# eritpchy/video-subtitle-extractor

Measured on AMD Instinct MI355X. Metric: OCR frames/sec (det+rec) @1080p, higher is better.
Workload: dtype f16

## Files before the change

### __graft_entry__.py

```python
import os
import subprocess
import sys

ROOT = os.path.dirname(os.path.abspath(__file__))
PKG = os.path.join(ROOT, "video-subtitle-extractor_amd")
CSRC = os.path.join(PKG, "csrc")
LIB = os.path.join(PKG, "libvse_hip.so")
HIP_SOURCES = ["vse_runtime.hip", "conv_select.hip", "conv_mfma.hip", "conv_gemm.hip", "conv_patch.hip", "conv_col.hip", "conv_c3.hip", "conv_pw.hip", "conv_dwpw.hip", "conv_smallm.hip", "conv_head.hip", "conv_stem.hip", "simple_ops.hip", "lstm.hip", "prepost.hip", "chain.hip", "frame_change.hip", "audio_match.hip"]


def _newer(target, deps):
    if not os.path.exists(target):
        return True
    t = os.path.getmtime(target)
    return any(os.path.getmtime(d) > t for d in deps)


def build(force=False):
    hipcc = os.environ.get("HIPCC", "/opt/rocm/bin/hipcc")
    srcs = [os.path.join(CSRC, s) for s in HIP_SOURCES]
    deps = srcs + [os.path.join(CSRC, "common.h"), os.path.join(CSRC, "conv_common.h"), os.path.join(CSRC, "db_geometry.h"),
                   os.path.join(ROOT, "include", "vse_hip.h")]
    if force or _newer(LIB, deps):
        objs = []
        os.makedirs(os.path.join(CSRC, "build"), exist_ok=True)
        procs = []
        for s in srcs:
            o = os.path.join(CSRC, "build", os.path.basename(s) + ".o")
            objs.append(o)
            if force or _newer(o, [s] + deps[len(srcs):]):
                cmd = [hipcc, "--offload-arch=gfx950", "-O3", "-std=c++17", "-fPIC", "-ffp-contract=off", "-c", s, "-o", o]
                procs.append((cmd, subprocess.Popen(cmd)))
        for cmd, p in procs:
            if p.wait() != 0:
                raise RuntimeError("hipcc failed: " + " ".join(cmd))
        cmd = [hipcc, "--offload-arch=gfx950", "-shared", "-fPIC", "-o", LIB] + objs
        subprocess.check_call(cmd)
    sys.path.insert(0, ROOT)
    import vse_amd
    from vse_amd import engine
    engine.load_library()
# ... 53 lines not shown
```

### video-subtitle-extractor_amd/csrc/conv_common.h

```cpp
#pragma once
#include "common.h"

#define PTW 32
#define CTW 32
#define CPW 48
#define C3BN 64
#define PW_MAXN 256
#define PW_MAXN_HILO 128
#define DWPW_ROWS_MAX_KS 3
#define DWPW_ROWS_MAX_KS_S1 3

struct ConvParams {
    const half_t* in;
    const half_t* w;
    const float* bias;
    const half_t* res;
    const half_t* zero;
    void* out;
    int H, W, Hs, Ws, in_ld, cinp, inshift;
    int OH, OW;
    long M;
    int kh, kw, sh, sw, ph, pw;
    int Np, nk;
    int nkh;
    int out_ld, out_f32;
    int res_ld, resshift, res_hs, res_ws;
    int act, act2;
    float act_a, act_b, post_a, post_b;
    int flags, coutp;
    unsigned ntn;
    unsigned ntiles;
    int tiles_h, tiles_w;
    const float* dotw;
    float dotb;
    int dotact, dot_f32, dot_ld;
    void* dot_out;
    const half_t* in2;
    int in2_ld, in2_shift, in2_hs, in2_ws, nv0;
    unsigned long long* trace;
    int vec16;
    long wimg_stride;
    int hw_img, tiles_img;
    const int* wl_out;
    int in_lo_off;
    int res_lo_off;
    int lo_off;
    const half_t* ogate;
    int ogate_ld;
    int wnp;
    const uint8_t* u8src;
    int u8_h, u8_w;
    long u8_pitch, u8_fstride;
    int pack_g, nimg;
    unsigned pack_mag_ow, pack_mag_d;
};

typedef const __attribute__((address_space(1))) void* gptr_t;
typedef __attribute__((address_space(3))) void* lptr_t;

__device__ __forceinline__ void glds16(const void* g, half_t* l) {
    __builtin_amdgcn_global_load_lds((gptr_t)g, (lptr_t)l, 16, 0, 0);
}

__device__ __forceinline__ void glds16_asm(const void* g, half_t* l) {
    unsigned keep;
    const unsigned dst = __builtin_amdgcn_readfirstlane((unsigned)(size_t)(lptr_t)l);
    asm volatile("s_mov_b32 %0, m0\n\ts_mov_b32 m0, %2\n\ts_nop 0\n\tglobal_load_lds_dwordx4 %1, off\n\ts_mov_b32 m0, %0"
                 : "=&s"(keep) : "v"(g), "s"(dst) : "memory");
}

#define OOB 0x80000000u
typedef __attribute__((address_space(3))) void* ldsv_t;

template <int N> __device__ __forceinline__ void wait_vm() {
    static_assert(N >= 0 && N <= 16, "vmcnt literal");
    if constexpr (N == 0) asm volatile("s_waitcnt vmcnt(0)" ::: "memory");
    else if constexpr (N == 1) asm volatile("s_waitcnt vmcnt(1)" ::: "memory");
    else if constexpr (N == 2) asm volatile("s_waitcnt vmcnt(2)" ::: "memory");
    else if constexpr (N == 3) asm volatile("s_waitcnt vmcnt(3)" ::: "memory");
    else if constexpr (N == 4) asm volatile("s_waitcnt vmcnt(4)" ::: "memory");
    else if constexpr (N == 5) asm volatile("s_waitcnt vmcnt(5)" ::: "memory");
    else if constexpr (N == 6) asm volatile("s_waitcnt vmcnt(6)" ::: "memory");
    else if constexpr (N == 7) asm volatile("s_waitcnt vmcnt(7)" ::: "memory");
    else if constexpr (N == 8) asm volatile("s_waitcnt vmcnt(8)" ::: "memory");
    else if constexpr (N == 9) asm volatile("s_waitcnt vmcnt(9)" ::: "memory");
    else if constexpr (N == 10) asm volatile("s_waitcnt vmcnt(10)" ::: "memory");
    else if constexpr (N == 11) asm volatile("s_waitcnt vmcnt(11)" ::: "memory");
// ... 167 lines not shown
    t.vlast = min(ox0 + TW, t.vw) - 1;
    t.g0 = (int)__umulhi((unsigned)ox0, p.pack_mag_ow);
    t.n0 = ox0 + p.pw * t.g0;
    t.used = TW + KW - 1 + p.pw * ((int)__umulhi((unsigned)max(t.vlast, 0), p.pack_mag_ow) - t.g0);
    return t;
}
__device__ __forceinline__ bool conv_pack_src(const ConvParams& p, const ConvPackTile& t, int px, int& g, int& ix) {
    const unsigned n = (unsigned)(t.n0 + px);
    g = (int)__umulhi(n, p.pack_mag_d);
    ix = (int)n - g * (p.W + p.pw) - p.pw;
    return px < t.used && ix >= 0 && ix < p.W && (long)g * p.OW < t.vw;
}
__device__ __forceinline__ int conv_pack_fragcol(const ConvParams& p, const ConvPackTile& t, int ox0, int v) {
    return v - ox0 + p.pw * ((int)__umulhi((unsigned)max(min(v, t.vlast), 0), p.pack_mag_ow) - t.g0);
}

__device__ __forceinline__ float conv_epilogue_dot(const ConvParams& p, const float16v& acc, const float (&bias)[16],
                                                   const float (&dotw)[16]) {
    float v[16];
#pragma unroll
    for (int e = 0; e < 16; ++e) v[e] = acc[e] + bias[e];
    vse_act_n(v, p.act, p.act_a, p.act_b);
    if (p.post_a != 1.f || p.post_b != 0.f) {
#pragma unroll
        for (int e = 0; e < 16; ++e) v[e] = v[e] * p.post_a + p.post_b;
    }
    vse_act_n(v, p.act2, 0.f, 0.f);
    float part = 0.f;
#pragma unroll
    for (int e = 0; e < 16; ++e) part += v[e] * dotw[e];
    return part;
}

enum { CK_NONE = 0, CK_GEMM, CK_SMALLM, CK_MFMA, CK_PATCH, CK_COL, CK_C3, CK_PW, CK_DWPW, CK_HEAD, CK_STEM };
struct ConvKernel {
    int family;
    int rc;
    int arg[3];
};

struct GemmCfg { int bm, bn, wm, wn, bk, st; };
constexpr GemmCfg kCfg[] = {{128, 128, 2, 2, 32, 3}, {256, 64, 4, 1, 32, 3}, {256, 32, 4, 1, 32, 3}, {256, 128, 4, 2, 32, 3},
                            {256, 256, 4, 4, 32, 3}, {256, 192, 8, 2, 32, 3}, {256, 256, 4, 4, 64, 2}, {256, 192, 8, 2, 64, 2}};

struct SrcGeom { int h, w; long pitch, fstride; };
ConvParams conv_params(const vse_op& o, const TView& in, const TView& res, const TView& in2, const TView& out, const TView& dot_out,
                       const char* wts, const half_t* zero, const int* wl_out, const uint8_t* u8src, const SrcGeom& src);
ConvKernel conv_select(const ConvParams& p, int Kp);
int conv_kernel_name(const ConvKernel& k, char* buf, size_t n);
int launch_conv(const vse_op& o, const TView& in, const TView& res, const TView& in2, const TView& out, const TView& dot_out,
                const char* wts, const half_t* zero, const int* wl_out, const uint8_t* u8src, const SrcGeom& src, hipStream_t st);
static inline long conv_images(const ConvParams& p) { return p.OH && p.OW ? p.M / ((long)p.OH * p.OW) : 0; }
int conv_pack_group(long images, int OW, int TW, int spare, int gap);
void conv_pack_plan(ConvParams& p, int TW, int spare);

int launch_conv_gemm(const ConvParams& p, const ConvKernel& k, hipStream_t st);
int launch_conv_smallm(const ConvParams& p, const ConvKernel& k, hipStream_t st);
int launch_conv_mfma(const ConvParams& p, const ConvKernel& k, hipStream_t st);
int launch_conv_patch(const ConvParams& p, const ConvKernel& k, hipStream_t st);
int launch_conv_col(const ConvParams& p, const ConvKernel& k, hipStream_t st);
int launch_conv_c3(const ConvParams& p, const ConvKernel& k, hipStream_t st);
int launch_conv_pw(const ConvParams& p, const ConvKernel& k, hipStream_t st);
int launch_conv_dwpw(const ConvParams& p, const ConvKernel& k, hipStream_t st);
int launch_conv_head(const ConvParams& p, const ConvKernel& k, hipStream_t st);
int launch_conv_stem(const ConvParams& p, const ConvKernel& k, hipStream_t st);
```

### video-subtitle-extractor_amd/csrc/conv_select.hip

```cpp
#include <stdlib.h>
#include <cstdio>
#include "conv_common.h"


static int conv_gemm_mode(int kh, int kw, int sh, int sw, int ph, int pw, int cinp, int Kp, int inshift, int flags) {
    (void)sh; (void)sw;
    if (inshift || (flags & (F_PATCH | F_DOT1 | F_SRC2))) return 0;
    if (cinp % 32) return 0;
    if (kh * kw > 31) return 0;
    if (kh < 2 * ph + 1 || kw < 2 * pw) return 0;
    if (kh == 1 && kw == 1 && ph == 0 && pw == 0 && Kp == cinp) return 2;
    return 1;
}
static bool conv_gemm_span_ok(const ConvParams& p, int Kp) {
    const double span = ((double)512 * p.sw + (512.0 / p.OW + 3) * p.sh * p.Ws + (double)p.kh * p.Ws + p.kw) * p.in_ld * 2;
    return !(span > 1.9e9 || (double)Kp * p.Np * 2 > 1.9e9);
}

static int conv_gemm_config(int Np, int cinp, long M) {
    auto ntn = [&](int bn) { return (long)((Np + bn - 1) / bn); };
    auto deep = [&](int c) { return cinp % 64 == 0 ? c + 2 : c; };
    if (Np <= 32) return 2;
    if (Np <= 64) return 1;
    const long mt = (M + 255) / 256;
// ... 225 lines not shown
    const int kt = (f & F_WK32) ? 32 : 64;
    const bool same_hw = p.H == p.OH && p.W == p.OW && p.Hs == p.H && p.Ws == p.W;
    if (conv_smallk_ok(p, same_hw)) return pick(CK_SMALLM, kt, hilo);
    const int mode = conv_gemm_mode(p.kh, p.kw, p.sh, p.sw, p.ph, p.pw, p.cinp, Kp, p.inshift, f);
    if (mode && conv_smallm_ok(p, mode, same_hw)) return pick(CK_SMALLM, kt, hilo);
    if (mode && conv_gemm_span_ok(p, Kp)) return pick(CK_GEMM, conv_gemm_config(p.Np, p.cinp, p.M), mode == 1);
    if (f & F_WK32) return refuse(VSE_E_UNSUPPORTED);
    return pick(CK_MFMA, conv_tile_bn(p.Np), p.inshift != 0);
}

int conv_kernel_name(const ConvKernel& k, char* buf, size_t n) {
    const int* a = k.arg;
    const char* tf[2] = {"false", "true"};
    if (k.rc != VSE_OK) return snprintf(buf, n, "(refused: %d)", k.rc);
    switch (k.family) {
        case CK_GEMM: {
            const GemmCfg& g = kCfg[a[0]];
            return snprintf(buf, n, "conv_gemm_kernel<%d, %d, %d, %d, %d, %d, %d>", g.bm, g.bn, g.wm, g.wn, g.bk, g.st, a[1]);
        }
        case CK_SMALLM: return snprintf(buf, n, "conv_smallm%s_kernel<%d>", a[1] ? "_hl" : "", a[0]);
        case CK_MFMA:
            return snprintf(buf, n, "conv_mfma_kernel<%d, %d, %d, %d, %s>", a[0] == 128 ? 128 : 256, a[0], a[0] == 128 ? 2 : 4, a[0] == 128 ? 2 : 1,
                            tf[a[1]]);
        case CK_PATCH: return snprintf(buf, n, "conv_patch_kernel<%d, %d, %d>", a[0], a[1], a[2]);
        case CK_COL: return snprintf(buf, n, "conv_col_kernel<%d, %d>", a[0], a[1]);
        case CK_C3: return snprintf(buf, n, "conv_c3%s_kernel<%d, %d>", a[1] ? "n32" : "", a[0], 8 / a[0]);
        case CK_PW:
            return a[2] ? snprintf(buf, n, "conv_pw_tail_kernel<%d>", a[0]) : snprintf(buf, n, "conv_pw_kernel<%d, %s>", a[0], tf[a[1]]);
        case CK_DWPW:
            return a[2] ? snprintf(buf, n, "conv_dwpw_rows_kernel<%d, %s, %d>", a[0], tf[a[1]], a[2])
                        : snprintf(buf, n, "conv_dwpw_kernel<%d, 3, %s>", a[0], tf[a[1]]);
        case CK_HEAD: return snprintf(buf, n, a[0] ? "conv_head_up2r_kernel" : "conv_head_up2_kernel");
        case CK_STEM: return snprintf(buf, n, "conv_stem_kernel<%d, %d, %s, %s>", a[0], a[0], tf[a[1]], tf[a[2]]);
        default: return snprintf(buf, n, "?");
    }
}


int launch_conv(const vse_op& o, const TView& in, const TView& res, const TView& in2, const TView& out, const TView& dot_out,
                const char* wts, const half_t* zero, const int* wl_out, const uint8_t* u8src, const SrcGeom& src, hipStream_t st) {
    const ConvParams p = conv_params(o, in, res, in2, out, dot_out, wts, zero, wl_out, u8src, src);
    const int f = p.flags, Np = p.Np, cinp = p.cinp;
    if (f & F_SRC2) {
        if (!in2.ptr || in2.esize != 2 || (in2.ld & 7) || in.c + in2.c != cinp) return VSE_E_INVAL;
        if ((in2.h << p.in2_shift) != p.H || (in2.w << p.in2_shift) != p.W) return VSE_E_INVAL;
    } else if (in.c != cinp) {
        return VSE_E_INVAL;
    }
    if (in.esize != 2 || ((in.ld & 7) && !((f & F_UP2HEAD) && in.ld == 1)) || (cinp & 7)) return VSE_E_INVAL;
    if ((f & F_RES) && (res.esize != 2 || (res.ld & 3))) return VSE_E_INVAL;
    if ((!(f & (F_DOT1 | F_ONECH)) && (out.ld & 3)) || (Np & 7)) return VSE_E_INVAL;
    if ((f & F_ONECH) && (!(f & F_PIXSHUF) || !(f & F_OUT_F32) || Np != 32 || out.ld != 1 || out.esize != 4 || (f & F_RES)))
        return VSE_E_INVAL;
    const int mul = (f & F_PIXSHUF) ? 2 : 1;
    if (out.h != p.OH * mul || out.w != p.OW * mul || out.n != in.n) return VSE_E_INVAL;
    if (p.res_lo_off && (!p.vec16 || p.resshift || (p.res_lo_off & 7))) return VSE_E_INVAL;
    if (p.lo_off && (!p.vec16 || (f & (F_OUT_F32 | F_ONECH | F_DOT1 | F_UP2HEAD)) || (p.lo_off & 7) || out.ld < p.lo_off + Np / ((f & F_PIXSHUF) ? 4 : 1)))
        return VSE_E_INVAL;
    if ((f & F_OGATE) && ((f & (F_SRC2 | F_IMGW | F_PIXSHUF | F_DOT1 | F_UP2HEAD)) || !in2.ptr || in2.esize != 2 || in2.n != in.n || in2.h != 1
                          || in2.w != 1 || in2.c < Np || (in2.ld & 7) || (reinterpret_cast<uintptr_t>(in2.ptr) & 15)))
        return VSE_E_INVAL;
    if ((f & F_U8SRC) && (!(f & F_STEM) || !p.u8src || p.u8_h <= 0 || p.u8_w <= 0)) return VSE_E_INVAL;
    if (p.wl_out && (f & (F_DOT1 | F_SRC2 | F_UP2HEAD | F_PIXSHUF))) return VSE_E_UNSUPPORTED;
    const ConvKernel k = conv_select(p, o.p[P_KTOT]);
    if (k.family == CK_NONE) return k.rc;
    if (!p.zero && !(f & (F_IMGW | F_DWPRE))) return VSE_E_INVAL;
    switch (k.family) {
        case CK_GEMM: return launch_conv_gemm(p, k, st);
// ... 12 lines not shown
```

### video-subtitle-extractor_amd/csrc/vse_runtime.hip

```cpp
#include <stdlib.h>
#include <cstdarg>
#include <cstdio>
#include <cstring>
#include <string>
#include <vector>

#include "conv_common.h"

static thread_local std::string g_err;
static void set_err(const char* fmt, ...) {
    char buf[512];
    va_list ap;
    va_start(ap, fmt);
    vsnprintf(buf, sizeof buf, fmt, ap);
    va_end(ap);
    g_err = buf;
}
void vse_set_error(const char* msg) { g_err = msg ? msg : ""; }
#define HIP_TRY(expr)                                                                  \
    do {                                                                               \
        hipError_t e_ = (expr);                                                        \
        if (e_ != hipSuccess) {                                                        \
            set_err("%s failed: %s (%s:%d)", #expr, hipGetErrorString(e_), __FILE__, __LINE__); \
            return VSE_E_HIP;                                                          \
        }                                                                              \
    } while (0)

struct vse_ctx {
    int device;
    std::vector<void*> weights;
    std::vector<size_t> weight_bytes;
    void* zero_page;
};

struct vse_plan {
    vse_ctx* ctx;
    int weights_id;
    std::vector<vse_op> ops;
    size_t ws_bytes;
    int max_ext;
    int n_levels;
    int batch;
    bool u8_source;
    int src_h, src_w;
    long src_pitch, src_fstride;
};

int vse_frame_change_launch(const void* d_bgr, int n, int64_t pitch, int64_t frame_stride, int y0, int y1, int x0, int x1, int edge_thresh,
                            void* d_state, int reset, int32_t* d_counts, void* stream);
size_t vse_audio_match_ws(const long* m, const long* n, int nq);
int vse_audio_match_launch(const uint8_t* const* pat, const uint8_t* const* win, const long* m, const long* n, int nq, void* d_ws,
                           unsigned long long* d_out, void* stream);

extern "C" {

const char* vse_last_error(void) { return g_err.c_str(); }
size_t vse_sizeof_op(void) { return sizeof(vse_op); }
size_t vse_sizeof_view(void) { return sizeof(vse_view); }
int vse_abi_version(void) { return 4; }

int vse_init(int device_id, vse_ctx** out) {
    if (!out) return VSE_E_INVAL;
    int count = 0;
    HIP_TRY(hipGetDeviceCount(&count));
    if (device_id < 0 || device_id >= count) {
        set_err("device %d not present (%d visible)", device_id, count);
        return VSE_E_INVAL;
    }
    HIP_TRY(hipSetDevice(device_id));
    hipDeviceProp_t prop;
    HIP_TRY(hipGetDeviceProperties(&prop, device_id));
// ... 85 lines not shown
            if (v->arena >= 2) p->max_ext = std::max(p->max_ext, v->arena - 2);
            if (v->arena == 0) {
                const size_t end = (size_t)v->off + ((size_t)v->n * v->h * v->w - 1) * v->ld * v->esize + (size_t)v->c * v->esize;
                if (end > ws_bytes) {
                    set_err("op %d: view exceeds workspace (%zu > %zu)", i, end, ws_bytes);
                    delete p;
                    return VSE_E_INVAL;
                }
            }
        }
        if ((size_t)o.w_off > wbytes || (size_t)o.b_off > wbytes) {
            set_err("op %d: weight offset out of range", i);
            delete p;
            return VSE_E_INVAL;
        }
        if (o.kind == OP_CHAIN) {
            int hdr[16];
            const size_t words = 16 + (size_t)std::max(o.p[4], 0) * 16 + (size_t)std::max(o.p[3], 0) * 28;
            if ((size_t)o.w_off + words * 4 > wbytes || (o.w_off & 3) ||
                hipMemcpy(hdr, reinterpret_cast<const char*>(c->weights[weights_id]) + o.w_off, sizeof hdr, hipMemcpyDeviceToHost) != hipSuccess) {
                set_err("op %d: chain descriptor out of the weight blob", i);
                delete p;
                return VSE_E_INVAL;
            }
            if (hdr[0] != 0x43484e31 || hdr[1] != o.p[3] || hdr[2] != o.p[4] || hdr[5] != o.p[2] || hdr[3] < 0 || hdr[4] < 0 ||
                (size_t)o.w_off + (size_t)hdr[4] + (size_t)hdr[3] > wbytes) {
                set_err("op %d: chain descriptor does not match its record (magic %#x, stages %d / %d, buffers %d / %d, LDS %d / %d)", i, hdr[0],
                        hdr[1], o.p[3], hdr[2], o.p[4], hdr[5], o.p[2]);
                delete p;
                return VSE_E_INVAL;
            }
        }
    }
    *out = p;
    return VSE_OK;
}

void vse_plan_destroy(vse_plan* p) { delete p; }

static inline TView resolve(const vse_view& v, char* ws, char* wts, void* const* ext) {
    TView t;
    t.ptr = nullptr;
    t.n = v.n; t.h = v.h; t.w = v.w; t.c = v.c; t.ld = v.ld; t.esize = v.esize;
    if (v.n == 0) return t;
    char* base = v.arena == 0 ? ws : (v.arena == 1 ? wts : reinterpret_cast<char*>(ext[v.arena - 2]));
    t.ptr = base + v.off;
    return t;
}

static int run_op(vse_plan* p, int i, char* ws, void* const* ext, const int32_t* wtab, hipStream_t st, const SrcGeom& src) {
    const vse_op& o = p->ops[i];
    const int* wl_in = (wtab && o.p[P_WLIN]) ? wtab + (size_t)(o.p[P_WLIN] - 1) * p->batch : nullptr;
    const int* wl_out = (wtab && o.p[P_WLOUT]) ? wtab + (size_t)(o.p[P_WLOUT] - 1) * p->batch : nullptr;
    char* wts = reinterpret_cast<char*>(p->ctx->weights[p->weights_id]);
    const TView in0 = resolve(o.in0, ws, wts, ext), in1 = resolve(o.in1, ws, wts, ext),
                in2 = resolve(o.in2, ws, wts, ext), out = resolve(o.out, ws, wts, ext),
                out2 = resolve(o.out2, ws, wts, ext);
    int rc;
    if (o.kind == OP_CONV) {
        const uint8_t* u8src = (o.flags & F_U8SRC) ? reinterpret_cast<const uint8_t*>(ext[0]) : nullptr;
        rc = launch_conv(o, in0, in1, in2, out, out2, wts, reinterpret_cast<const half_t*>(p->ctx->zero_page), wl_out, u8src, src, st);
    } else if (o.kind == OP_CHAIN) {
        rc = launch_chain(o, in0, out, out2, in2, wts, st);
    } else {
        rc = launch_simple_op(o, in0, in1, in2, out, out2, wts, wl_in, wl_out, st);
    }
    if (rc != VSE_OK) set_err("op %d (kind %d) failed to launch: rc=%d (%s)", i, o.kind, rc, hipGetErrorString(hipGetLastError()));
    return rc;
}

static int check_run(vse_plan* p, void* ws, void* const* ext, int n_ext, const int32_t* d_widths, const char* who) {
    if (!p || !ext || n_ext <= p->max_ext) {
        set_err("%s: need %d external pointers", who, p ? p->max_ext + 1 : 0);
        return VSE_E_INVAL;
    }
    if (!ws && p->ws_bytes) return VSE_E_INVAL;
    if (p->n_levels && !d_widths) {
        set_err("%s: the plan was compiled for ragged batches (%d width levels): run it with a width table", who, p->n_levels);
        return VSE_E_INVAL;
    }
    if (!p->n_levels && d_widths) {
        set_err("%s: width table given to a plan that was not compiled for ragged batches", who);
        return VSE_E_INVAL;
    }
    if (p->u8_source && (p->src_h <= 0 || p->src_w <= 0)) {
        set_err("%s: the plan pre-processes the uint8 frames in its stem: call vse_plan_set_source (or vse_det_forward) first", who);
        return VSE_E_INVAL;
    }
    return VSE_OK;
}

int vse_plan_set_source(vse_plan* p, int src_h, int src_w, int64_t pitch, int64_t frame_stride) {
// ... 199 lines not shown
    static thread_local char buf[96];
    buf[0] = 0;
    if (!op) return buf;
    const vse_op& o = *op;
    static const char* simple[] = {"", "", "dwconv_kernel", "pool_kernel", "gap_kernel", "scale_kernel", "binary_kernel", "resize_kernel",
                                   "unary_kernel", "layernorm_kernel", "attn_kernel", "softmax_kernel", "lstm_kernel", "wscale_kernel", "chain_kernel"};
    if (o.kind != OP_CONV) {
        snprintf(buf, sizeof buf, "%s", (o.kind >= 2 && o.kind <= OP_CHAIN) ? simple[o.kind] : "?");
        return buf;
    }
    auto shape = [](const vse_view& v) { return TView{nullptr, v.n, v.h, v.w, v.c, v.ld, v.esize}; };
    const ConvParams p = conv_params(o, shape(o.in0), shape(o.in1), shape(o.in2), shape(o.out), shape(o.out2), nullptr, nullptr, nullptr, nullptr,
                                     SrcGeom{0, 0, 0, 0});
    conv_kernel_name(conv_select(p, o.p[P_KTOT]), buf, sizeof buf);
    return buf;
}

int vse_plan_profile(vse_plan* p, void* ws, void* const* ext, int n_ext, const int32_t* d_widths, void* stream, float* ms) {
    if (!ms) return VSE_E_INVAL;
    int rc0 = check_run(p, ws, ext, n_ext, d_widths, "vse_plan_profile");
    if (rc0 != VSE_OK) return rc0;
    hipStream_t st = reinterpret_cast<hipStream_t>(stream);
    const int n = (int)p->ops.size();
    std::vector<hipEvent_t> ev(n + 1);
    for (auto& e : ev) HIP_TRY(hipEventCreate(&e));
    HIP_TRY(hipEventRecord(ev[0], st));
    for (int i = 0; i < n; ++i) {
        int rc = run_op(p, i, reinterpret_cast<char*>(ws), ext, d_widths, st, SrcGeom{p->src_h, p->src_w, p->src_pitch, p->src_fstride});
        if (rc != VSE_OK) return rc;
        HIP_TRY(hipEventRecord(ev[i + 1], st));
    }
    HIP_TRY(hipStreamSynchronize(st));
    for (int i = 0; i < n; ++i) HIP_TRY(hipEventElapsedTime(&ms[i], ev[i], ev[i + 1]));
    for (auto& e : ev) (void)hipEventDestroy(e);
    return VSE_OK;
}

}
```

### video-subtitle-extractor_amd/engine.py

```python
import ctypes as C
import os

import numpy as np

from . import compiler, ir

_HERE = os.path.dirname(os.path.abspath(__file__))
LIB_PATH = os.environ.get("VSE_LIB_PATH") or os.path.join(_HERE, "libvse_hip.so")

EXPORTS = [
    "vse_init", "vse_destroy", "vse_last_error", "vse_sizeof_op", "vse_sizeof_view", "vse_abi_version",
    "vse_weights_upload", "vse_weights_free", "vse_plan_create", "vse_plan_destroy", "vse_plan_run", "vse_plan_run_ragged",
    "vse_plan_width_levels", "vse_plan_profile", "vse_op_kernel_name", "vse_det_preprocess", "vse_db_workspace_bytes",
    "vse_db_postprocess", "vse_rec_preprocess", "vse_rec_preprocess_scratch_bytes", "vse_ctc_collapse", "vse_ctc_collapse_ragged",
    "vse_det_forward", "vse_rec_forward", "vse_plan_set_source", "vse_plan_takes_frames",
    "vse_rec_graph_create", "vse_graph_launch", "vse_graph_destroy", "vse_frame_change_state_bytes", "vse_frame_change",
    "vse_audio_match_workspace_bytes", "vse_audio_match",
]


class VseError(RuntimeError):
    pass


# ... 70 lines not shown
                                       C.c_void_p]
    lib.vse_db_postprocess.argtypes = [C.c_void_p, C.c_void_p, C.c_int, C.c_int, C.c_int, C.c_int, C.c_int,
                                       C.POINTER(DbParams), C.c_void_p, C.c_size_t, C.POINTER(Box), C.c_int,
                                       C.POINTER(C.c_int), C.c_void_p]
    lib.vse_rec_preprocess.argtypes = [C.c_void_p, C.c_void_p, C.c_int, C.c_int, C.c_int, C.c_int64, C.c_int64,
                                       C.POINTER(Crop), C.c_int, C.c_void_p, C.c_int, C.c_int, C.c_void_p,
                                       C.c_size_t, C.c_void_p]
    lib.vse_ctc_collapse.argtypes = [C.c_void_p, C.c_void_p, C.c_int, C.c_int, C.c_void_p, C.c_void_p, C.c_void_p,
                                     C.c_void_p]
    lib.vse_ctc_collapse_ragged.argtypes = [C.c_void_p, C.c_void_p, C.c_int, C.c_int, C.c_void_p, C.c_void_p, C.c_void_p,
                                            C.c_void_p, C.c_void_p]
    lib.vse_frame_change_state_bytes.restype = C.c_size_t
    lib.vse_frame_change_state_bytes.argtypes = [C.c_int, C.c_int]
    lib.vse_frame_change.argtypes = [C.c_void_p, C.c_void_p, C.c_int, C.c_int, C.c_int, C.c_int64, C.c_int64, C.c_int, C.c_int,
                                     C.c_int, C.c_int, C.c_int, C.c_void_p, C.c_int, C.c_void_p, C.c_void_p]
    lib.vse_audio_match_workspace_bytes.restype = C.c_size_t
    lib.vse_audio_match_workspace_bytes.argtypes = [C.c_void_p, C.c_int]
    lib.vse_audio_match.argtypes = [C.c_void_p, C.c_void_p, C.c_int64, C.c_void_p, C.c_int64, C.c_void_p, C.c_int, C.c_void_p,
                                    C.c_size_t, C.c_void_p, C.c_void_p]
    if lib.vse_sizeof_op() != ir.OP_DT.itemsize or lib.vse_sizeof_view() != ir.VIEW_DT.itemsize:
        raise VseError(f"ABI mismatch: vse_op {lib.vse_sizeof_op()} vs {ir.OP_DT.itemsize}, "
                       f"vse_view {lib.vse_sizeof_view()} vs {ir.VIEW_DT.itemsize}")
    _lib = lib
    return lib


def op_kernel_names(ops):
    lib = load_library()
    ops = np.ascontiguousarray(ops)
    base = ops.ctypes.data
    return [lib.vse_op_kernel_name(C.c_void_p(base + i * ops.itemsize)).decode() for i in range(len(ops))]


def _check(rc, what):
    if rc < 0:
        raise VseError(f"{what} failed (rc={rc}): {load_library().vse_last_error().decode(errors='replace')}")
    return rc


def _torch():
    import torch
    if not torch.cuda.is_available():
        raise VseError("no HIP device visible: the OCR hot path runs only on MI355X (gfx950); no CPU fallback")
    return torch


class Context:

    def __init__(self, device=0):
        self.lib = load_library()
        self.torch = _torch()
        self.device = device
        self.handle = C.c_void_p()
        _check(self.lib.vse_init(device, C.byref(self.handle)), "vse_init")
        self.tdev = self.torch.device("cuda", device)

    def stream(self):
        return C.c_void_p(self.torch.cuda.current_stream(self.tdev).cuda_stream)

    def streams_concurrent(self, a, b, spin_cycles=1_500_000):
        t = self.torch
        x = self.__dict__.setdefault("_probe_buf", t.zeros(64, device=self.tdev))
        for s in (a, b):
            with t.cuda.stream(s):
                x.add_(1)
        t.cuda.synchronize(self.tdev)
# ... 328 lines not shown

    def det_forward(self, frames_u8, dst_h, dst_w, slot=0):
        t = self.ctx.torch
        assert frames_u8.dtype == t.uint8 and frames_u8.dim() == 4 and frames_u8.shape[3] == 3
        assert frames_u8.stride(3) == 1 and frames_u8.stride(2) == 3
        n, h, w, _ = frames_u8.shape
        self.program(n, dst_h, dst_w)
        prog, handle = self._ensure((n, dst_h, dst_w))
        assert len(prog.outputs) == 1 and prog.outputs[0]["kind"] == "map" and prog.outputs[0]["ld"] == 1, "not a one-map detector plan"
        x = None if self.fuse_preprocess else t.empty((n, dst_h, dst_w, 8), dtype=t.float16, device=self.ctx.tdev)
        prob = t.empty((n, dst_h, dst_w), dtype=t.float32, device=self.ctx.tdev)
        ws = self._workspace((n, dst_h, dst_w), prog, slot)
        _check(self.ctx.lib.vse_det_forward(self.ctx.handle, handle, C.c_void_p(ws.data_ptr()), C.c_void_p(frames_u8.data_ptr()), n, h, w,
                                            frames_u8.stride(1), frames_u8.stride(0), dst_h, dst_w, 1 if self.input_norm is not None else 0,
                                            C.c_void_p(x.data_ptr()) if x is not None else None, C.c_void_p(prob.data_ptr()),
                                            self.ctx.stream()), "vse_det_forward")
        return prob

    def profile_frames(self, frames_u8, dst_h, dst_w, slot=0):
        if not self.fuse_preprocess:
            return self.profile(self.ctx.det_preprocess(frames_u8, dst_h, dst_w, raw=self.input_norm is not None), slot)
        t = self.ctx.torch
        n, h, w, _ = frames_u8.shape
        self.program(n, dst_h, dst_w)
        prog, handle = self._ensure((n, dst_h, dst_w))
        _check(self.ctx.lib.vse_plan_set_source(handle, h, w, frames_u8.stride(1), frames_u8.stride(0)), "vse_plan_set_source")
        outs = [t.empty((o["n"], o["h"], o["w"], o["ld"]), dtype=t.float32, device=self.ctx.tdev) for o in prog.outputs]
        ptrs = (C.c_void_p * (1 + len(outs)))(frames_u8.data_ptr(), *[o.data_ptr() for o in outs])
        ms = (C.c_float * len(prog.ops))()
        ws = self._workspace((n, dst_h, dst_w), prog, slot)
        self.last_outs = outs
        _check(self.ctx.lib.vse_plan_profile(handle, C.c_void_p(ws.data_ptr()), ptrs, len(ptrs), None, self.ctx.stream(), ms),
               "vse_plan_profile")
        names = op_kernel_names(prog.ops)
        return np.array(ms[:], dtype=np.float32), prog, names

    def rec_forward(self, x, widths=None, slot=0):
        t = self.ctx.torch
        assert x.dtype == t.float16 and x.is_contiguous() and x.shape[3] == 8
        n, h, w, _ = x.shape
        self.program(n, h, w)
        prog, handle = self._ensure((n, h, w))
        assert len(prog.outputs) == 1 and prog.outputs[0]["kind"] == "idx_maxp"
        tt = prog.outputs[0]["w"]
        wt = self._width_table(prog, widths, n, w)
        idx_maxp = t.empty((n, 1, tt, 2), dtype=t.float32, device=self.ctx.tdev)
        oi = t.zeros((n, tt), dtype=t.int32, device=self.ctx.tdev)
        ol = t.empty((n,), dtype=t.int32, device=self.ctx.tdev)
        oc = t.empty((n,), dtype=t.float32, device=self.ctx.tdev)
        ws = self._workspace((n, h, w), prog, slot)
        _check(self.ctx.lib.vse_rec_forward(self.ctx.handle, handle, C.c_void_p(ws.data_ptr()), C.c_void_p(x.data_ptr()),
                                            C.c_void_p(wt.data_ptr()) if wt is not None else None, prog.out_level,
                                            C.c_void_p(idx_maxp.data_ptr()), n, tt, C.c_void_p(oi.data_ptr()), C.c_void_p(ol.data_ptr()),
                                            C.c_void_p(oc.data_ptr()), self.ctx.stream()), "vse_rec_forward")
        return oi, ol, oc

    def rec_graph_buffers(self, n, h, w, slot=0):
        t = self.ctx.torch
        key = (n, h, w, slot)
        if not hasattr(self, "_graphs"):
            self._graphs = {}
        if key in self._graphs:
            self._graphs[key] = self._graphs.pop(key)
        else:
            self._drop_graphs(keep=self.GRAPH_CACHE_MAX - 1)
            self.program(n, h, w)
            prog, handle = self._ensure((n, h, w))
# ... 5 lines not shown
                ol=t.zeros((n,), dtype=t.int32, device=dev), oc=t.zeros((n,), dtype=t.float32, device=dev), graph=None, tt=tt,
                wsbuf=t.zeros(max(prog.ws_bytes, 256), dtype=t.uint8, device=dev), prog=prog, handle=handle)
        return self._graphs[key]

    def rec_forward_graph(self, bufs, widths):
        t = self.ctx.torch
        prog = bufs["prog"]
        self._upload_i32(prog.width_table(widths), out=bufs["wt"])
        if bufs["graph"] is None:
            g = C.c_void_p()
            n = bufs["x"].shape[0]
            _check(self.ctx.lib.vse_rec_graph_create(self.ctx.handle, bufs["handle"], C.c_void_p(bufs["wsbuf"].data_ptr()),
                                                     C.c_void_p(bufs["x"].data_ptr()), C.c_void_p(bufs["wt"].data_ptr()), prog.out_level,
                                                     C.c_void_p(bufs["idx_maxp"].data_ptr()), n, bufs["tt"], C.c_void_p(bufs["oi"].data_ptr()),
                                                     C.c_void_p(bufs["ol"].data_ptr()), C.c_void_p(bufs["oc"].data_ptr()), self.ctx.stream(),
                                                     C.byref(g)), "vse_rec_graph_create")
            bufs["graph"] = g
        _check(self.ctx.lib.vse_graph_launch(bufs["graph"], self.ctx.stream()), "vse_graph_launch")
        return bufs["oi"].clone(), bufs["ol"].clone(), bufs["oc"].clone()

    def profile(self, x, slot=0, widths=None):
        n, h, w, _ = x.shape
        self.program(n, h, w)
        prog, handle = self._ensure((n, h, w))
        outs, ptrs = self._ext(prog, x)
        ms = (C.c_float * len(prog.ops))()
        ws = self._workspace((n, h, w), prog, slot)
        wt = self._width_table(prog, widths, n, w)
        self.last_tlen = wt[prog.out_level] if wt is not None else None
        self.last_outs = outs
        _check(self.ctx.lib.vse_plan_profile(handle, C.c_void_p(ws.data_ptr()), ptrs, len(ptrs),
                                             C.c_void_p(wt.data_ptr()) if wt is not None else None, self.ctx.stream(), ms),
               "vse_plan_profile")
        variants = op_kernel_names(prog.ops)
        return np.array(ms[:], dtype=np.float32), prog, variants
```

Baseline: 2058.

## Fuse 3x3 conv with following 3x3 stride-2 max pool into one kernel

New measurement: 2088, median of 6. +1.5%, better.

```diff
diff --git a/__graft_entry__.py b/__graft_entry__.py
--- a/__graft_entry__.py
+++ b/__graft_entry__.py
@@ -6,7 +6,7 @@
 PKG = os.path.join(ROOT, "video-subtitle-extractor_amd")
 CSRC = os.path.join(PKG, "csrc")
 LIB = os.path.join(PKG, "libvse_hip.so")
-HIP_SOURCES = ["vse_runtime.hip", "conv_select.hip", "conv_mfma.hip", "conv_gemm.hip", "conv_patch.hip", "conv_col.hip", "conv_c3.hip", "conv_pw.hip", "conv_dwpw.hip", "conv_smallm.hip", "conv_head.hip", "conv_stem.hip", "simple_ops.hip", "lstm.hip", "prepost.hip", "chain.hip", "frame_change.hip", "audio_match.hip"]
+HIP_SOURCES = ["vse_runtime.hip", "conv_select.hip", "conv_mfma.hip", "conv_gemm.hip", "conv_patch.hip", "conv_col.hip", "conv_c3.hip", "conv_c3pool.hip", "conv_pw.hip", "conv_dwpw.hip", "conv_smallm.hip", "conv_head.hip", "conv_stem.hip", "simple_ops.hip", "lstm.hip", "prepost.hip", "chain.hip", "frame_change.hip", "audio_match.hip"]
 
 
 def _newer(target, deps):
diff --git a/video-subtitle-extractor_amd/csrc/conv_c3pool.hip b/video-subtitle-extractor_amd/csrc/conv_c3pool.hip
--- /dev/null
+++ b/video-subtitle-extractor_amd/csrc/conv_c3pool.hip
@@ -0,0 +1,244 @@
+#include "conv_common.h"
+
+template <int BN>
+__global__ __launch_bounds__(512, 4) void conv_c3pool_kernel(const ConvParams p) {
+    constexpr int PTH = 8, WCO = 2;
+    constexpr int TN = BN / (32 * WCO);
+    constexpr int PPIX = 352, PNPL = 3, TPS = 2, RING = 2;
+    constexpr int PW = PTW + 2, P = PW * (PTH + 2);
+    constexpr int PATCH_HALFS = PPIX * 32, WSTAGE_HALFS = TPS * BN * 32, DUMMY_HALFS = 2 * 512;
+    constexpr int NCG = BN / 8;
+    static_assert(BN == 64 || BN == 128, "cout tile");
+    static_assert(PTH * PTW * BN <= 2 * PATCH_HALFS + RING * WSTAGE_HALFS + DUMMY_HALFS, "the fp16 conv tile must fit the patch + ring");
+    __shared__ __attribute__((aligned(16))) half_t lds[2 * PATCH_HALFS + RING * WSTAGE_HALFS + DUMMY_HALFS + 2 * BN];
+    float* const sbias = reinterpret_cast<float*>(lds + 2 * PATCH_HALFS + RING * WSTAGE_HALFS + DUMMY_HALFS);
+    half_t* const patch0 = lds;
+    half_t* const ring0 = lds + 2 * PATCH_HALFS;
+    half_t* const dummy0 = ring0 + RING * WSTAGE_HALFS;
+
+    const int tid = threadIdx.x;
+    const int lane = tid & 63;
+    const int wave = __builtin_amdgcn_readfirstlane(tid >> 6);
+    const int wpx = wave / WCO, wco = wave % WCO;
+
+    const unsigned nblk = gridDim.x, bid = blockIdx.x;
+    const unsigned q8 = nblk >> 3, r8 = nblk & 7, xcd = bid & 7, slot = bid >> 3;
+    unsigned t = (xcd < r8 ? xcd * (q8 + 1) : r8 * (q8 + 1) + (xcd - r8) * q8) + slot;
+    const int nt = t % p.ntn;  t /= p.ntn;
+    const int tx = t % p.tiles_w;  t /= p.tiles_w;
+    const int seg = t % p.pool_nseg;
+    const long img = t / p.pool_nseg;
+    const int ox0 = tx * (PTW - 2) - 1, n0 = nt * BN;
+    const int ty_first = seg * p.pool_seg, ty_end = min(ty_first + p.pool_seg, p.tiles_h);
+    const int PHp = (p.OH - 1) / 2 + 1, PWp = (p.OW - 1) / 2 + 1;
+
+    const int nchunks = (p.cinp + 31) >> 5;
+    const int taps = p.kh * p.kw, pairs = (taps + TPS - 1) / TPS;
+
+    const int kv = (lane & 3) ^ ((lane >> 4) & 3);
+    const int wr = BN == 128 ? (tid >> 2) : ((tid >> 2) & 63);
+    const bool wok = n0 + wr < p.Np;
+    const long winc = wok ? (long)p.Np * 32 * TPS : 0;
+
+    const int fx = lane & 31, fj = lane >> 5;
+    unsigned woffb[TN];
+#pragma unroll
+    for (int j = 0; j < TN; ++j) {
+        const int r = wco * (BN / WCO) + j * 32 + conv_wrow(fx);
+        woffb[j] = (unsigned)(r * 64 + ((fj ^ ((r >> 2) & 3)) << 4));
+    }
+    const int qb0 = (2 * wpx) * PW + fx, qb1 = qb0 + PW;
+    const char* const ring_b = reinterpret_cast<const char*>(ring0);
+
+    const half_t lowest = (half_t)-65504.f;
+    const half8 lowest8 = {lowest, lowest, lowest, lowest, lowest, lowest, lowest, lowest};
+    half8 carry = lowest8;
+
+    conv_stage_consts<true>(sbias, p.bias, p.zero, n0, BN, p.Np, wave, lane);
+
+    for (int ty = ty_first > 0 ? ty_first - 1 : 0; ty < ty_end; ++ty) {
+        const int oy0 = ty * PTH;
+        int ptid = tid, twave = wave;
+        asm volatile("" : "+v"(ptid), "+s"(twave));
+        long poff[PNPL];
+        bool pok[PNPL];
+#pragma unroll
+        for (int j = 0; j < PNPL; ++j) {
+            const int q = 16 * (twave + 8 * j) + ((ptid & 63) >> 2);
+            const int py = q / PW, px = q - py * PW;
+            const int iy = oy0 - 1 + py, ix = ox0 - 1 + px;
+            pok[j] = (q < P) && (iy >= 0) && (iy < p.H) && (ix >= 0) && (ix < p.W);
+            poff[j] = ((img * p.Hs + iy) * p.Ws + ix) * (long)p.in_ld + ((ptid & 3) ^ ((ptid >> 4) & 3)) * 8;
+        }
+        const int pwr = BN == 128 ? (ptid >> 2) : ((ptid >> 2) & 63);
+        const half_t* wptr = n0 + pwr < p.Np ? p.w + (long)(n0 + pwr) * 32 + ((ptid & 3) ^ ((ptid >> 4) & 3)) * 8
+                                                   + (BN == 128 ? 0 : (long)(twave >> 2) * p.Np * 32)
+                                             : p.zero;
+        auto issue_patch = [&](int cc, int buf) {
+            half_t* base = patch0 + buf * PATCH_HALFS;
+            const bool live = (cc < nchunks) && (cc * 32 + kv * 8 < p.cinp);
+#pragma unroll
+            for (int j = 0; j < PNPL; ++j) {
+                const half_t* src = p.zero;
+                if (live && pok[j]) src = p.in + poff[j] + cc * 32;
+                half_t* dst = base + (twave + 8 * j) * 16 * 32;
+                if (j == PNPL - 1 && twave >= 6) { src = p.zero; dst = dummy0 + (twave - 6) * 512; }
+                glds16_asm(src, dst);
+            }
+        };
+        auto issue_w = [&](int s) {
+            half_t* st = ring0 + (s & (RING - 1)) * WSTAGE_HALFS;
+            if constexpr (BN == 128) {
+                glds16_asm(wptr, st + twave * 16 * 32);
+                glds16_asm(wptr + (wok ? (long)p.Np * 32 : 0), st + BN * 32 + twave * 16 * 32);
+            } else {
+                glds16_asm(wptr, st + (twave >> 2) * BN * 32 + (twave & 3) * 16 * 32);
+            }
+            wptr += winc;
+        };
+        const bool wave_live = (oy0 + 2 * wpx) < p.OH && (ty >= ty_first || wpx == PTH / 2 - 1);
+
+        float16v acc[2][TN];
+#pragma unroll
+        for (int i = 0; i < 2; ++i)
+#pragma unroll
+            for (int j = 0; j < TN; ++j)
+#pragma unroll
+                for (int r = 0; r < 16; ++r) acc[i][j][r] = 0.f;
+
+        issue_patch(0, 0);
+        issue_w(0);
+
+        int s = 0;
+        for (int cc = 0; cc < nchunks; ++cc) {
+            const char* const pb = reinterpret_cast<const char*>(patch0 + (cc & 1) * PATCH_HALFS);
+            const bool klim1 = (p.cinp - cc * 32) <= 16;
+            int tapoff = 0, dx = 0, dy = 0, tap = 0;
+            half8 xc[2];
+            xc[0] = xc[1] = half8{0, 0, 0, 0, 0, 0, 0, 0};
+            for (int pr = 0; pr < pairs; ++pr, ++s) {
+                if (pr == 1) asm volatile("s_waitcnt vmcnt(3)" ::: "memory");
+                else asm volatile("s_waitcnt vmcnt(0)" ::: "memory");
+                __builtin_amdgcn_s_barrier();
+                asm volatile("" ::: "memory");
+                issue_w(s + 1);
+                if (pr == 0) issue_patch(cc + 1, (cc + 1) & 1);
+                const unsigned wsb = (unsigned)(s & (RING - 1)) * (WSTAGE_HALFS * 2);
+#pragma unroll
+                for (int h = 0; h < TPS; ++h) {
+                    if (h >= 1 && tap >= taps) break;
+                    const unsigned q0 = (unsigned)(qb0 + tapoff), q1 = (unsigned)(qb1 + tapoff);
+                    const unsigned a0 = (q0 << 6) + ((fj ^ ((q0 >> 2) & 3)) << 4), a1 = (q1 << 6) + ((fj ^ ((q1 >> 2) & 3)) << 4);
+#pragma unroll
+                    for (int ks = 0; ks < 2; ++ks) {
+                        if (!wave_live) break;
+                        if (ks == 1 && klim1) break;
+                        half8 wf[TN], xf[2];
+#pragma unroll
+                        for (int j = 0; j < TN; ++j)
+                            wf[j] = *reinterpret_cast<const half8*>(ring_b + wsb + h * (BN * 64) + (woffb[j] ^ (ks << 5)));
+                        if (dy == 0) xf[0] = *reinterpret_cast<const half8*>(pb + (a0 ^ (ks << 5)));
+                        else xf[0] = xc[ks];
+                        xf[1] = *reinterpret_cast<const half8*>(pb + (a1 ^ (ks << 5)));
+                        xc[ks] = xf[1];
+#pragma unroll
+                        for (int i = 0; i < 2; ++i)
+#pragma unroll
+                            for (int j = 0; j < TN; ++j)
+                                acc[i][j] = __builtin_amdgcn_mfma_f32_32x32x16_f16(wf[j], xf[i], acc[i][j], 0, 0, 0);
+                    }
+                    if (++tap < taps) {
+                        if (++dy == p.kh) { dy = 0; tapoff = ++dx; } else { tapoff += PW; }
+                    }
+                }
+            }
+        }
+        asm volatile("s_waitcnt vmcnt(0)" ::: "memory");
+        __syncthreads();
+
+        int elane = lane;
+        asm volatile("" : "+v"(elane));
+        const int ex = elane & 31, ej = elane >> 5;
+#pragma unroll
+        for (int i = 0; i < 2; ++i) {
+            half_t* const px = lds + ((2 * wpx + i) * PTW + ex) * BN;
+#pragma unroll
+            for (int j = 0; j < TN; ++j) {
+                float bias[16], v[16];
+                conv_epilogue_consts(sbias, wco * (BN / WCO) + j * 32, elane, bias);
+#pragma unroll
+                for (int e = 0; e < 16; ++e) v[e] = acc[i][j][e] + bias[e];
+                vse_act_n(v, p.act, p.act_a, p.act_b);
+                if (p.post_a != 1.f || p.post_b != 0.f) {
+#pragma unroll
+                    for (int e = 0; e < 16; ++e) v[e] = v[e] * p.post_a + p.post_b;
+                }
+                vse_act_n(v, p.act2, 0.f, 0.f);
+#pragma unroll
+                for (int g = 0; g < 2; ++g) {
+                    const int c8 = (wco * (BN / WCO) + j * 32 + g * 16 + ej * 8) >> 3;
+                    const float* w = v + g * 8;
+                    *reinterpret_cast<half8*>(px + ((c8 ^ (ex & (NCG - 1))) << 3)) =
+                        half8{(half_t)w[0], (half_t)w[1], (half_t)w[2], (half_t)w[3], (half_t)w[4], (half_t)w[5], (half_t)w[6], (half_t)w[7]};
+                }
+            }
+        }
+        __syncthreads();
+
+        int qtid = tid;
+        asm volatile("" : "+v"(qtid));
+        const int cg = qtid & (NCG - 1), pc = (qtid / NCG) & 15, rp = (qtid / (NCG * 16)) & 1;
+        if (qtid < NCG * 32 && pc < 15) {
+            auto colmax = [&](int r) {
+                half8 m = lowest8;
+                if (oy0 + r >= p.OH) return m;
+#pragma unroll
+                for (int dc = 0; dc < 3; ++dc) {
+                    const int lc = 2 * pc + dc, gx = ox0 + lc;
+                    if (gx < 0 || gx >= p.OW) continue;
+                    m = __builtin_elementwise_max(m, *reinterpret_cast<const half8*>(lds + (r * PTW + lc) * BN + ((cg ^ (lc & (NCG - 1))) << 3)));
+                }
+                return m;
+            };
+            const int rb = 4 * rp;
+            const half8 e = colmax(rp ? 3 : 7);
+            const half8 first = rp ? e : carry;
+            const half8 a = colmax(rb), b = colmax(rb + 1), c = colmax(rb + 2), d = colmax(rb + 3);
+            carry = rp ? carry : e;
+            const int pcol = tx * 15 + pc, prow = 4 * ty + 2 * rp;
+            if (ty >= ty_first && pcol < PWp && n0 + cg * 8 < p.Np) {
+                half_t* const op = reinterpret_cast<half_t*>(p.out) + ((img * PHp + prow) * PWp + pcol) * (long)p.out_ld + n0 + cg * 8;
+                if (prow < PHp) *reinterpret_cast<half8*>(op) = __builtin_elementwise_max(__builtin_elementwise_max(first, a), b);
+                if (prow + 1 < PHp)
+                    *reinterpret_cast<half8*>(op + (long)PWp * p.out_ld) = __builtin_elementwise_max(__builtin_elementwise_max(b, c), d);
+            }
+        }
+        __syncthreads();
+    }
+}
+
+static void conv_c3pool_strips(long images, int tiles_h, int tiles_w, int ntn, int* seg, int* nseg) {
+    int n = 1;
+    while (images * tiles_w * ntn * n < 1024 && (tiles_h + n) / (n + 1) >= 4) ++n;
+    *seg = (tiles_h + n - 1) / n;
+    *nseg = (tiles_h + *seg - 1) / *seg;
+}
+
+int launch_conv_c3pool(const ConvParams& pin, const ConvKernel& k, hipStream_t st) {
+    ConvParams p = pin;
+    if (p.kh != 3 || p.kw != 3 || p.sh != 1 || p.sw != 1 || p.ph != 1 || p.pw != 1 || (p.cinp & 7) || p.inshift || p.OH != p.H || p.OW != p.W)
+        return VSE_E_INVAL;
+    if ((p.flags & ~F_PATCH) || p.out_f32 || p.lo_off || p.wl_out || (p.out_ld & 7) || (reinterpret_cast<uintptr_t>(p.out) & 15) || (p.Np & 7))
+        return VSE_E_INVAL;
+    const int bn = k.arg[0];
+    p.ntn = (unsigned)((p.Np + bn - 1) / bn);
+    p.tiles_h = (p.OH + 7) / 8;
+    p.tiles_w = ((p.OW - 1) / 2 + 1 + 14) / 15;
+    conv_c3pool_strips(conv_images(p), p.tiles_h, p.tiles_w, (int)p.ntn, &p.pool_seg, &p.pool_nseg);
+    const unsigned long long blocks = (unsigned long long)conv_images(p) * p.pool_nseg * p.tiles_w * p.ntn;
+    if (blocks == 0 || blocks > 0x7fffffffull) return VSE_E_INVAL;
+    const dim3 grid((unsigned)blocks), block(512);
+    if (bn == 128) hipLaunchKernelGGL((conv_c3pool_kernel<128>), grid, block, 0, st, p);
+    else hipLaunchKernelGGL((conv_c3pool_kernel<64>), grid, block, 0, st, p);
+    return hipGetLastError() == hipSuccess ? VSE_OK : VSE_E_HIP;
+}
diff --git a/video-subtitle-extractor_amd/csrc/conv_common.h b/video-subtitle-extractor_amd/csrc/conv_common.h
--- a/video-subtitle-extractor_amd/csrc/conv_common.h
+++ b/video-subtitle-extractor_amd/csrc/conv_common.h
@@ -53,6 +53,7 @@
     long u8_pitch, u8_fstride;
     int pack_g, nimg;
     unsigned pack_mag_ow, pack_mag_d;
+    int pool_seg, pool_nseg;
 };
 
 typedef const __attribute__((address_space(1))) void* gptr_t;
@@ -286,7 +287,7 @@
     return part;
 }
 
-enum { CK_NONE = 0, CK_GEMM, CK_SMALLM, CK_MFMA, CK_PATCH, CK_COL, CK_C3, CK_PW, CK_DWPW, CK_HEAD, CK_STEM };
+enum { CK_NONE = 0, CK_GEMM, CK_SMALLM, CK_MFMA, CK_PATCH, CK_COL, CK_C3, CK_PW, CK_DWPW, CK_HEAD, CK_STEM, CK_C3POOL };
 struct ConvKernel {
     int family;
     int rc;
@@ -304,6 +305,9 @@
 int conv_kernel_name(const ConvKernel& k, char* buf, size_t n);
 int launch_conv(const vse_op& o, const TView& in, const TView& res, const TView& in2, const TView& out, const TView& dot_out,
                 const char* wts, const half_t* zero, const int* wl_out, const uint8_t* u8src, const SrcGeom& src, hipStream_t st);
+ConvKernel conv_pool_select(const vse_op* ops, int n_ops, int i);
+int launch_conv_pool(const vse_op& conv, const ConvKernel& k, const TView& in, const TView& pool_out, const char* wts, const half_t* zero,
+                     hipStream_t st);
 static inline long conv_images(const ConvParams& p) { return p.OH && p.OW ? p.M / ((long)p.OH * p.OW) : 0; }
 int conv_pack_group(long images, int OW, int TW, int spare, int gap);
 void conv_pack_plan(ConvParams& p, int TW, int spare);
@@ -314,6 +318,7 @@
 int launch_conv_patch(const ConvParams& p, const ConvKernel& k, hipStream_t st);
 int launch_conv_col(const ConvParams& p, const ConvKernel& k, hipStream_t st);
 int launch_conv_c3(const ConvParams& p, const ConvKernel& k, hipStream_t st);
+int launch_conv_c3pool(const ConvParams& p, const ConvKernel& k, hipStream_t st);
 int launch_conv_pw(const ConvParams& p, const ConvKernel& k, hipStream_t st);
 int launch_conv_dwpw(const ConvParams& p, const ConvKernel& k, hipStream_t st);
 int launch_conv_head(const ConvParams& p, const ConvKernel& k, hipStream_t st);
diff --git a/video-subtitle-extractor_amd/csrc/conv_select.hip b/video-subtitle-extractor_amd/csrc/conv_select.hip
--- a/video-subtitle-extractor_amd/csrc/conv_select.hip
+++ b/video-subtitle-extractor_amd/csrc/conv_select.hip
@@ -281,8 +281,63 @@
                         : snprintf(buf, n, "conv_dwpw_kernel<%d, 3, %s>", a[0], tf[a[1]]);
         case CK_HEAD: return snprintf(buf, n, a[0] ? "conv_head_up2r_kernel" : "conv_head_up2_kernel");
         case CK_STEM: return snprintf(buf, n, "conv_stem_kernel<%d, %d, %s, %s>", a[0], a[0], tf[a[1]], tf[a[2]]);
+        case CK_C3POOL: return snprintf(buf, n, "conv_c3pool_kernel<%d>", a[0]);
         default: return snprintf(buf, n, "?");
     }
+}
+
+
+static void view_span(const vse_view& v, int64_t* lo, int64_t* hi) {
+    *lo = v.off;
+    *hi = v.off + (((int64_t)v.n * v.h * v.w - 1) * v.ld + v.c) * v.esize;
+}
+static bool views_overlap(const vse_view& a, const vse_view& b) {
+    if (a.n == 0 || b.n == 0 || a.arena != b.arena) return false;
+    int64_t a0, a1, b0, b1;
+    view_span(a, &a0, &a1);
+    view_span(b, &b0, &b1);
+    return a0 < b1 && b0 < a1;
+}
+static bool same_view(const vse_view& a, const vse_view& b) {
+    return a.off == b.off && a.arena == b.arena && a.n == b.n && a.h == b.h && a.w == b.w && a.c == b.c && a.ld == b.ld && a.esize == b.esize;
+}
+
+ConvKernel conv_pool_select(const vse_op* ops, int n_ops, int i) {
+    const ConvKernel no{CK_NONE, VSE_OK, {0, 0, 0}};
+    if (!ops || i < 0 || i + 1 >= n_ops) return no;
+    const vse_op &c = ops[i], &q = ops[i + 1];
+    if (c.kind != OP_CONV || q.kind != OP_POOL) return no;
+    if (c.flags != F_PATCH || c.p[P_KH] != 3 || c.p[P_KW] != 3 || c.p[P_SH] != 1 || c.p[P_SW] != 1 || c.p[P_PH] != 1 || c.p[P_PW] != 1) return no;
+    if (c.p[P_INSHIFT] || c.p[P_LO_OUT] || c.p[P_WLIN] || c.p[P_WLOUT] || q.p[P_WLIN] || q.p[P_WLOUT]) return no;
+    if (c.in1.n || c.in2.n || c.out2.n || q.in1.n || q.in2.n || q.out2.n) return no;
+    if (!q.p[P_POOL_MAX] || q.p[P_KH] != 3 || q.p[P_KW] != 3 || q.p[P_SH] != 2 || q.p[P_SW] != 2 || q.p[P_PH] != 1 || q.p[P_PW] != 1) return no;
+    if (c.out.arena != 0 || c.out.esize != 2 || c.in0.esize != 2 || !same_view(c.out, q.in0)) return no;
+    if (c.out.n != c.in0.n || c.out.h != c.in0.h || c.out.w != c.in0.w || c.out.c != c.p[P_COUT] || (c.p[P_COUT] & 7)) return no;
+    if (q.out.esize != 2 || q.out.n != c.out.n || q.out.h != (c.out.h - 1) / 2 + 1 || q.out.w != (c.out.w - 1) / 2 + 1 || q.out.c != c.out.c ||
+        (q.out.ld & 7) || (q.out.off & 15))
+        return no;
+    if (views_overlap(c.in0, q.out) || views_overlap(c.out, q.out) || views_overlap(c.out, c.in0)) return no;
+    int th, bn, mode;
+    conv_patch_plan(3, 3, c.out.h, c.p[P_COUT], c.flags, &th, &bn, &mode);
+    if (mode != 2) return no;
+    for (int j = i + 2; j < n_ops; ++j) {
+        const vse_op& o = ops[j];
+        if (views_overlap(o.in0, c.out) || views_overlap(o.in1, c.out) || views_overlap(o.in2, c.out) || views_overlap(o.out2, c.out)) return no;
+        if (views_overlap(o.out, c.out)) break;
+    }
+    return ConvKernel{CK_C3POOL, VSE_OK, {bn, 0, 0}};
+}
+
+int launch_conv_pool(const vse_op& conv, const ConvKernel& k, const TView& in, const TView& pool_out, const char* wts, const half_t* zero,
+                     hipStream_t st) {
+    if (k.family != CK_C3POOL || !in.ptr || !pool_out.ptr || !zero) return VSE_E_INVAL;
+    const TView none{nullptr, 0, 0, 0, 0, 0, 0};
+    const TView shape{nullptr, conv.out.n, conv.out.h, conv.out.w, conv.out.c, conv.out.ld, conv.out.esize};
+    ConvParams p = conv_params(conv, in, none, none, shape, none, wts, zero, nullptr, nullptr, SrcGeom{0, 0, 0, 0});
+    if (in.c != p.cinp || (in.ld & 7)) return VSE_E_INVAL;
+    p.out = pool_out.ptr;
+    p.out_ld = pool_out.ld;
+    return launch_conv_c3pool(p, k, st);
 }
 
 
diff --git a/video-subtitle-extractor_amd/csrc/vse_runtime.hip b/video-subtitle-extractor_amd/csrc/vse_runtime.hip
--- a/video-subtitle-extractor_amd/csrc/vse_runtime.hip
+++ b/video-subtitle-extractor_amd/csrc/vse_runtime.hip
@@ -37,6 +37,7 @@
     vse_ctx* ctx;
     int weights_id;
     std::vector<vse_op> ops;
+    std::vector<ConvKernel> pooled;
     size_t ws_bytes;
     int max_ext;
     int n_levels;
@@ -188,6 +189,8 @@
             }
         }
     }
+    p->pooled.assign(n_ops, ConvKernel{CK_NONE, VSE_OK, {0, 0, 0}});
+    for (int i = 0; i + 1 < n_ops && !p->n_levels; ++i) p->pooled[i] = conv_pool_select(ops, n_ops, i);
     *out = p;
     return VSE_OK;
 }
@@ -213,7 +216,11 @@
                 in2 = resolve(o.in2, ws, wts, ext), out = resolve(o.out, ws, wts, ext),
                 out2 = resolve(o.out2, ws, wts, ext);
     int rc;
-    if (o.kind == OP_CONV) {
+    if (i > 0 && p->pooled[i - 1].family == CK_C3POOL) return VSE_OK;
+    if (p->pooled[i].family == CK_C3POOL) {
+        const TView pool_out = resolve(p->ops[i + 1].out, ws, wts, ext);
+        rc = launch_conv_pool(o, p->pooled[i], in0, pool_out, wts, reinterpret_cast<const half_t*>(p->ctx->zero_page), st);
+    } else if (o.kind == OP_CONV) {
         const uint8_t* u8src = (o.flags & F_U8SRC) ? reinterpret_cast<const uint8_t*>(ext[0]) : nullptr;
         rc = launch_conv(o, in0, in1, in2, out, out2, wts, reinterpret_cast<const half_t*>(p->ctx->zero_page), wl_out, u8src, src, st);
     } else if (o.kind == OP_CHAIN) {
@@ -479,6 +486,8 @@
     }
     HIP_TRY(hipStreamSynchronize(st));
     for (int i = 0; i < n; ++i) HIP_TRY(hipEventElapsedTime(&ms[i], ev[i], ev[i + 1]));
+    for (int i = 1; i < n; ++i)
+        if (p->pooled[i - 1].family == CK_C3POOL) ms[i] = 0.f;
     for (auto& e : ev) (void)hipEventDestroy(e);
     return VSE_OK;
 }
diff --git a/video-subtitle-extractor_amd/engine.py b/video-subtitle-extractor_amd/engine.py
--- a/video-subtitle-extractor_amd/engine.py
+++ b/video-subtitle-extractor_amd/engine.py
@@ -126,6 +126,15 @@
     return [lib.vse_op_kernel_name(C.c_void_p(base + i * ops.itemsize)).decode() for i in range(len(ops))]
 
 
+def profiled_kernel_names(ops, ms):
+    names = op_kernel_names(ops)
+    for i in range(1, len(names)):
+        if (int(ops[i]["kind"]) == ir.OP_POOL and int(ops[i - 1]["kind"]) == ir.OP_CONV and float(ms[i]) == 0.0
+                and names[i - 1].startswith("conv_patch_kernel<")):
+            names[i - 1] = "conv_c3pool_kernel<%s>" % names[i - 1].split(",")[1].strip()
+    return names
+
+
 def _check(rc, what):
     if rc < 0:
         raise VseError(f"{what} failed (rc={rc}): {load_library().vse_last_error().decode(errors='replace')}")
@@ -520,7 +529,7 @@
         self.last_outs = outs
         _check(self.ctx.lib.vse_plan_profile(handle, C.c_void_p(ws.data_ptr()), ptrs, len(ptrs), None, self.ctx.stream(), ms),
                "vse_plan_profile")
-        names = op_kernel_names(prog.ops)
+        names = profiled_kernel_names(prog.ops, ms)
         return np.array(ms[:], dtype=np.float32), prog, names
 
     def rec_forward(self, x, widths=None, slot=0):
@@ -592,5 +601,5 @@
         _check(self.ctx.lib.vse_plan_profile(handle, C.c_void_p(ws.data_ptr()), ptrs, len(ptrs),
                                              C.c_void_p(wt.data_ptr()) if wt is not None else None, self.ctx.stream(), ms),
                "vse_plan_profile")
-        variants = op_kernel_names(prog.ops)
+        variants = profiled_kernel_names(prog.ops, ms)
         return np.array(ms[:], dtype=np.float32), prog, variants
```
